# PKU-EPIC/GraspNeRF

Hardware: AMD Instinct MI355X
Metric: scenes/sec TSDF+render fwd, 6-view 40^3 grid (higher is better)
Workload: dtype f32

## Files before the change

graspnerf_amd/csrc/gnr_kernels.hip:

```cpp
#include <hip/hip_runtime.h>
#include <stdint.h>
#include <type_traits>

#include "gnr_layout.h"

#ifndef GNR_ABLATE
#define GNR_ABLATE 0
#endif

namespace gnr {

typedef float f4 __attribute__((ext_vector_type(4)));
typedef float f2 __attribute__((ext_vector_type(2)));

#define DEV __device__ __forceinline__

DEV f4 mfma16(float a, float b, f4 c) { return __builtin_amdgcn_mfma_f32_16x16x4f32(a, b, c, 0, 0, 0); }
DEV float elu1(float x) { return fmaxf(x, __builtin_amdgcn_fmed3f(__expf(x), 0.f, 1.f) - 1.f); }
constexpr float kLog2e = 1.4426950408889634f, kLn2 = 0.6931471805599453f;
#if GNR_ABLATE & 8
DEV float elu_s(float xs) { return xs; }
#else
DEV float elu_s(float xs) { return fmaxf(xs, fmaf(__builtin_amdgcn_fmed3f(__builtin_amdgcn_exp2f(xs), 0.f, 1.f), kLog2e, -kLog2e)); }
#endif
// ... 689 lines not shown
        return t < t_end - xcd * chunk ? xcd * chunk + t : -1;
#endif
    };
    auto locate = [&](int tile_, int& b_, int& ts_) {
        b_ = tile_ / tps;
        ts_ = tile_ - b_ * tps;
        b_ += a.b0;
        if (a.vol_res > 0) {
            const int R = a.vol_res, tpg = R >> 3, gpr = R >> 1;
            const int BX = R >> 2, GY = R >> 3, GB = BX * GY;
            const int sidx = ts_ / tpg, tin = ts_ - sidx * tpg;
            const int brick = sidx / GB, wi = sidx - brick * GB;
            const int bx = brick >> 2, by = brick & 3;
            ts_ = ((BX * bx + wi / GY) * gpr + GY * by + wi % GY) * tpg + tin;
        }
    };
    auto point_of = [&](int b_, int ts_) -> size_t { const int nr = ts_ * 16 + r; return (size_t)b_ * a.P + (nr < a.P ? nr : a.P - 1); };
    int tile = dyn ? resolve(grab()) : xcd * chunk + lblk * waves_per_block + wave;
    constexpr bool DPF = GNR_DESC_PREFETCH != 0 && !SAVE;
    f4 d0n = {0.f, 0.f, 0.f, 0.f}, d1n = d0n;
    bool have_nxt = false;
    for (; dyn ? tile >= 0 : tile < t_end;) {
        GNR_ITER_FENCE();
        unsigned tile_nxt = 0u;
        int tile_after = -1;
#if GNR_WAVE_CLOCK
        const unsigned long long wc_tt = wall_clock64();
#endif
        int b, ts;
        locate(tile, b, ts);
        const int n_raw = ts * 16 + r;
        const bool row_ok = n_raw < a.P;
        const int n = row_ok ? n_raw : a.P - 1;
        const size_t pt = (size_t)b * a.P + n;
        size_t opt = pt;
        if (RENDER && !SAVE && a.ray_perm) {
            const int s_ = n / a.perm_dn;
            opt = (size_t)b * a.P + (size_t)a.ray_perm[(size_t)b * a.perm_rn + s_] * a.perm_dn + (n - s_ * a.perm_dn);
        }
        float p[3], qd[3], lo, hi;
        {
            f4 d0, d1;
            if (DPF && have_nxt) { d0 = d0n; d1 = d1n; }
            else if (!RENDER && !SAVE && GNR_VOLUME_POINTS_INLINE != 0 && a.pts_R > 0) {
                const int R = a.pts_R;
                const float invR = 1.f / (float)R;
                const int col = (int)(((float)n + 0.5f) * invR), sz = n - col * R;
                const int ix = (int)(((float)col + 0.5f) * invR), iy = col - ix * R, iz = R - 1 - sz;
                const double vs = 0.3 / (double)R, hv = vs / 2;
                const float* bm = a.bbox_min + b * 3;
                d0 = (f4){(float)(ix * vs + hv) + bm[0], (float)(iy * vs + hv) + bm[1], (float)(iz * vs + hv) + bm[2], 0.f};
                d1 = (f4){0.f, 1.f, 0.005f, 0.005f};
            }
            else { d0 = reinterpret_cast<const f4*>(a.desc)[pt * 2]; d1 = reinterpret_cast<const f4*>(a.desc)[pt * 2 + 1]; }
            p[0] = d0.x; p[1] = d0.y; p[2] = d0.z; qd[0] = d0.w; qd[1] = d1.x; qd[2] = d1.y; lo = d1.z; hi = d1.w;
        }
        constexpr int VA = rows_a(V), VB = rows_b(V);
        float SA[VA][SW], SB[VB > 0 ? VB : 1][SW];
        auto S = [&](int v, int q) -> float& { return (VB == 0 || v < VA) ? SA[v < VA ? v : 0][q] : SB[v >= VA ? v - VA : 0][q]; };
#pragma unroll
        for (int k = 0; k < V; ++k)
#pragma unroll
#if GNR_ABLATE & 1
            for (int q = 0; q < SW; ++q) S(k, q) = p[0] * (float)(k * SW + q + 1);
#else
            for (int q = 0; q < SW; ++q) S(k, q) = 0.f;
#endif
        float msum = 0.f;
        unsigned vbits = 0;
#if GNR_ABLATE & 2
        ViewGeom vg0;
        project_view<true>(a.viewp + b * V * VIEWP_FLOATS, p, qd, a.H, a.W, vg0);
        const Taps t0 = make_taps(vg0.u, vg0.v, fsx, fsy, -0.5f, a.fh, a.fw);
        const Taps ti0 = make_taps(vg0.u, vg0.v, 1.f, 1.f, 0.f, a.H, a.W);
#endif

        auto phase1 = [&](auto& Q, const int v0) __attribute__((always_inline)) {
          constexpr int NQ = (int)(sizeof(Q) / sizeof(Q[0]));
#pragma unroll 1
          for (int v = v0; v < v0 + NQ; ++v) {
#if !(GNR_ABLATE & 1)
#pragma unroll
            for (int k = 0; k < NQ - 1; ++k)
#pragma unroll
                for (int q = 0; q < SW; ++q) Q[k][q] = Q[k + 1][q];
#endif
            GNR_ITER_FENCE();
            float (&Sv)[SW] = Q[NQ - 1];
            const int bv = b * V + v;
            const float* vp = a.viewp + bv * VIEWP_FLOATS;
            ViewGeom vg;
            Taps t, ti;
#if GNR_ABLATE & 2
            vg = vg0; t = t0; ti = ti0;
#elif GNR_COOP_PROJ
            {
                CoopOut co;
                project_coop(vp, lds + COOP_TAB + g * 8, (g & 1) * 16, (lane & 15) << 2, p, co);
                view_dir(vp, p, qd, vg.dd);
                vg.z = co.z; vg.m = co.m; t = co.f; ti = co.i;
            }
#else
            project_view<true>(vp, p, qd, a.H, a.W, vg);
            t = make_taps(vg.u, vg.v, fsx, fsy, -0.5f, a.fh, a.fw);
            ti = make_taps(vg.u, vg.v, 1.f, 1.f, 0.f, a.H, a.W);
#endif
            const float m = vg.m;
            msum += m;
            vbits |= (m != 0.f ? 1u : 0u) << v;
#if GNR_SKIP_MASKED
            if constexpr (!SAVE && RENDER) {
                if (__ballot(m != 0.f) == 0ull) {
#pragma unroll
                    for (int q = 0; q < SW; ++q) Sv[q] = 0.f;
                    if (a.dbg && g == 0 && row_ok) { a.dbg[pt * 32 + v] = 0.f; a.dbg[pt * 32 + 8 + v] = 0.f; }
                    continue;
                }
            }
#endif

            float FR[8], XI[9];
            {
                const float* fb = a.feat64 + (size_t)bv * a.fh * a.fw * 64 + 8 * g;
                const f4* q00 = reinterpret_cast<const f4*>(fb + (size_t)t.o00 * 64);
                const f4* q01 = reinterpret_cast<const f4*>(fb + (size_t)t.o01 * 64);
                const f4* q10 = reinterpret_cast<const f4*>(fb + (size_t)t.o10 * 64);
                const f4* q11 = reinterpret_cast<const f4*>(fb + (size_t)t.o11 * 64);
                const float w00 = t.w00 * m, w01 = t.w01 * m, w10 = t.w10 * m, w11 = t.w11 * m;
#pragma unroll
                for (int h = 0; h < 2; ++h) {
                    const f4 a0 = q00[h], a1 = q01[h], a2 = q10[h], a3 = q11[h];
                    const f4 c0 = q00[8 + h], c1 = q01[8 + h], c2 = q10[8 + h], c3 = q11[8 + h];
                    const f4 fr = a0 * w00 + a1 * w01 + a2 * w10 + a3 * w11;
                    const f4 fi = c0 * w00 + c1 * w01 + c2 * w10 + c3 * w11;
                    FR[4 * h] = fr.x; FR[4 * h + 1] = fr.y; FR[4 * h + 2] = fr.z; FR[4 * h + 3] = fr.w;
                    XI[4 * h] = fi.x; XI[4 * h + 1] = fi.y; XI[4 * h + 2] = fi.z; XI[4 * h + 3] = fi.w;
                }
                const float* ib = a.imgs + ((size_t)bv * 3 + min(g, 2)) * a.H * a.W;
                const float rgb = (ib[ti.o00] * ti.w00 + ib[ti.o01] * ti.w01 + ib[ti.o10] * ti.w10 + ib[ti.o11] * ti.w11) * m;
                XI[8] = g < 3 ? rgb : 0.f;
            }
            Sv[19] = XI[8];

            float o5[5];
            P8 frp;
            if constexpr (SP) frp = split8<0>(FR);
#pragma unroll
            for (int br = 0; br < 3; ++br) {
                f4 acc[2];
                float h1[8], h2[8];
                load_bias<2, LF>(lds + LO(pk::B_DEC1) + br * 32, g, acc);
                if constexpr (SP) mm16<1, 2, LF>(lds + LO(pk::DEC1) + br * frag_floats(8, 2), lane, &frp, acc);
                else mm<8, 2, 0, LF>(lds + LO(pk::DEC1) + br * frag_floats(8, 2), lane, FR, acc);
                elu_to<2, !SP>(acc, h1);
                load_bias<2, LF>(lds + LO(pk::B_DEC2) + br * 32, g, acc);
                if constexpr (SP) {
                    if constexpr (UA) { const P8U hp = split8u<0>(h1); mm16u<1, 2, LF, true>(lds + LO(pk::DEC2) + br * frag_floats(8, 2), lane, &hp, acc, &msum); }
                    else { const P8 hp = split8<0>(h1); mm16<1, 2, LF, true>(lds + LO(pk::DEC2) + br * frag_floats(8, 2), lane, &hp, acc, &msum); }
                }
                else mm<8, 2, 0, LF>(lds + LO(pk::DEC2) + br * frag_floats(8, 2), lane, h1, acc);
                elu_to<2, !SP || UA>(acc, h2);
                if (br < 2) {
                    o5[2 * br] = gsum(dot8(lds + LO(pk::T_DEC3) + (2 * br) * 32, g, h2)) + lds[LO(pk::T_DEC3_B) + 2 * br];
                    o5[2 * br + 1] = gsum(dot8(lds + LO(pk::T_DEC3) + (2 * br + 1) * 32, g, h2)) + lds[LO(pk::T_DEC3_B) + 2 * br + 1];
                } else {
                    o5[4] = gsum(dot8(lds + LO(pk::T_DEC3) + 4 * 32, g, h2)) + lds[LO(pk::T_DEC3_B) + 4];
                }
            }
            float hit, vis;
            {
                const bool m1 = (g & 1) != 0, far_edge = g >= 2;
                const float meang = softplus1(m1 ? o5[1] : o5[0]);
                const float varg = softplus1(m1 ? o5[3] : o5[2]) + 0.05f;
                const float mix = sigmoid1(m1 ? -o5[4] : o5[4]);
                const float dinv = -rcp1(fmaxf(vg.z, 1e-5f));
                const float dhat = (dinv - vp[15]) * vp[17];
                const float edge = far_edge ? dhat + hi : dhat - lo;
                float cg = 0.5f + 0.5f * tanh1((edge - meang) * varg);
                if constexpr (USEVIS) {
                    f4 acc[2];
                    float h1[8], h2[8];
                    load_bias<2, LF>(lds + LO(pk::B_DECV1), g, acc);
                    if constexpr (SP) mm16<1, 2, LF>(lds + LO(pk::DECV1), lane, &frp, acc);
                    else mm<8, 2, 0, LF>(lds + LO(pk::DECV1), lane, FR, acc);
                    elu_to<2, !SP>(acc, h1);
                    load_bias<2, LF>(lds + LO(pk::B_DECV2), g, acc);
                    if constexpr (SP) {
                        if constexpr (UA) { const P8U hp = split8u<0>(h1); mm16u<1, 2, LF, true>(lds + LO(pk::DECV2), lane, &hp, acc, &msum); }
                        else { const P8 hp = split8<0>(h1); mm16<1, 2, LF, true>(lds + LO(pk::DECV2), lane, &hp, acc, &msum); }
                    }
                    else mm<8, 2, 0, LF>(lds + LO(pk::DECV2), lane, h1, acc);
                    elu_to<2, !SP || UA>(acc, h2);
                    const float pv = sigmoid1(gsum(dot8(lds + LO(pk::T_DECV3), g, h2)) + lds[LO(pk::T_VIS)]);
                    cg *= pv;
                }
                const float mc = mix * cg;
                vis = gsum(far_edge ? 0.f : mix - mc) * m;
                hit = gsum(far_edge ? mc : -mc) * m;
            }
            {
                f4 acc[2];
                float e1[8];
                load_bias<2, LF>(lds + LO(pk::B_PE1), g, acc);
                if constexpr (SP) mm16<1, 2, LF>(lds + LO(pk::PE1), lane, &frp, acc);
                else mm<8, 2, 0, LF>(lds + LO(pk::PE1), lane, FR, acc);
                const float extra[1] = {g == 0 ? (hit - 0.5f) * 2.f : (g == 1 ? (vis - 0.5f) * 2.f : 0.f)};
                mm<1, 2, 8, LF>(lds + LO(pk::PE1), lane, extra, acc);
#pragma unroll
                for (int nb = 0; nb < 2; ++nb) {
                    e1[nb * 4 + 0] = fmaxf(acc[nb].x, 0.f); e1[nb * 4 + 1] = fmaxf(acc[nb].y, 0.f);
                    e1[nb * 4 + 2] = fmaxf(acc[nb].z, 0.f); e1[nb * 4 + 3] = fmaxf(acc[nb].w, 0.f);
                }
                if constexpr (EP) p8_store(split8<0>(e1), &Sv[9]);
                else {
#pragma unroll
                    for (int j = 0; j < 8; ++j) Sv[9 + j] = e1[j];
                }
            }
            {
                f4 acc1[1], acc3[3];
                float d1[4], df[12];
                load_bias<1, LF>(lds + LO(pk::B_RDF1), g, acc1);
                const float ddg[1] = {g == 0 ? vg.dd[0] : (g == 1 ? vg.dd[1] : (g == 2 ? vg.dd[2] : vg.dd[3]))};
                mm<1, 1, 0, LF>(lds + LO(pk::RDF1), lane, ddg, acc1);
                elu_to<1, true>(acc1, d1);
                load_bias<3, LF>(lds + LO(pk::B_RDF2), g, acc3);
#if GNR_RDF2_PAIRS
                if constexpr (SP && !USEVIS) { const P8 dp = split8z<0, 4>(d1); mm16<1, 3, LF>(lds + pk::c16_off(pk::DECV1), lane, &dp, acc3); }
                else
#endif
                mm<4, 3, 0, LF>(lds + LO(pk::RDF2), lane, d1, acc3);
                elu_to<3, true>(acc3, df);
#pragma unroll
                for (int j = 0; j < 9; ++j) Sv[j] = fmaf(df[j], kLn2, XI[j]);
            }
            {
                f4 acc1[1];
                float e[8], n1[4];
#pragma unroll
                for (int j = 0; j < 8; ++j) e[j] = Sv[9 + j];
                load_bias<1, LF>(lds + LO(pk::B_NR1), g, acc1);
                if constexpr (SP) { const P8 ep = EP ? p8_load(e) : split8<0>(e); mm16<1, 1, LF, true>(lds + LO(pk::NR1), lane, &ep, acc1, &msum); }
                else mm<8, 1, 0, LF>(lds + LO(pk::NR1), lane, e, acc1);
                elu_to<1, !SP>(acc1, n1);
                Sv[17] = sigmoid1(gsum(dot4(lds + LO(pk::T_NR2), g, n1)) + lds[LO(pk::T_SCAL) + 0]);
            }
            Sv[18] = m;
            if (SAVE && a.save1) {
                float* sp = a.save1 + (((size_t)b * tps + ts) * V + v) * 19 * 64 + lane;
#pragma unroll
                for (int q = 0; q < 19; ++q) sp[q * 64] = Sv[q];
            }
            if (a.dbg && g == 0 && row_ok) { a.dbg[pt * 32 + v] = hit; a.dbg[pt * 32 + 8 + v] = vis; }
          }
        };
        phase1(SA, 0);
        if constexpr (VB > 0) phase1(SB, VA);
#if GNR_WAVE_CLOCK
        const unsigned long long wc_p1 = wall_clock64();
#endif

        float SV[36];
        const float inv_msum = rcp1(msum + 1e-8f);
        {
#pragma unroll
            for (int j = 0; j < 9; ++j) {
                float mu0 = 0.f, mu1 = 0.f;
#pragma unroll
                for (int v = 0; v < V; ++v) {
                    const float w = S(v, 18) * inv_msum;
                    mu0 += S(v, j) * (S(v, 17) * w);
                    mu1 += S(v, j) * w;
                }
                float va0 = 0.f, va1 = 0.f;
#pragma unroll
                for (int v = 0; v < V; ++v) {
                    const float w = S(v, 18) * inv_msum;
                    const float d0 = S(v, j) - mu0, d1 = S(v, j) - mu1;
                    va0 += (S(v, 17) * w) * d0 * d0;
                    va1 += w * d1 * d1;
                }
                SV[j] = mu0; SV[9 + j] = va0; SV[18 + j] = mu1; SV[27 + j] = va1;
            }
        }
        f4 G[4];
        load_bias<4, LF>(lds + LO(pk::B_HOIST), g, G);
        if constexpr (SP) {
            const P8 sp[5] = {split8<0>(SV), split8<8>(SV), split8<16>(SV), split8<24>(SV), split8z<32, 4>(SV)};
            mm16<5, 4, LF, true>(lds + LO(pk::HOIST), lane, sp, G, &msum);
        } else mm<36, 4, 0, LF>(lds + LO(pk::HOIST), lane, SV, G);
        if (SAVE && a.saveG) {
            float* sp = a.saveG + ((size_t)b * tps + ts) * 17 * 64 + lane;
#pragma unroll
            for (int nb = 0; nb < 4; ++nb) {
                sp[(4 * nb) * 64] = G[nb].x; sp[(4 * nb + 1) * 64] = G[nb].y; sp[(4 * nb + 2) * 64] = G[nb].z; sp[(4 * nb + 3) * 64] = G[nb].w;
            }
            sp[16 * 64] = inv_msum;
        }

#if GNR_WAVE_CLOCK
        const unsigned long long wc_p2 = wall_clock64();
#endif
        float vsum = 0.f;
        auto phase2 = [&](auto& Q, const int v0) __attribute__((always_inline)) {
          constexpr int NQ = (int)(sizeof(Q) / sizeof(Q[0]));
#pragma unroll 1
          for (int v = v0; v < v0 + NQ; ++v) {
            constexpr int RN = 20;
            float Rv[RN];
#pragma unroll
            for (int j = 0; j < RN; ++j) Rv[j] = Q[0][j];
#if !(GNR_ABLATE & 1)
#pragma unroll
            for (int k = 0; k < NQ - 1; ++k)
#pragma unroll
                for (int q = 0; q < SW; ++q) Q[k][q] = Q[k + 1][q];
#endif
            GNR_ITER_FENCE();
            float X[9], E[8];
#pragma unroll
            for (int j = 0; j < 9; ++j) X[j] = Rv[j];
#pragma unroll
            for (int j = 0; j < 8; ++j) E[j] = Rv[9 + j];
            const float m = Rv[18];
            const float w = m * inv_msum;
#if GNR_SKIP_MASKED
            if constexpr (!SAVE && RENDER) {
                if (__ballot(m != 0.f) == 0ull) {
#pragma unroll
                    for (int j = 0; j < 9; ++j) Q[NQ - 1][j] = 0.f;
                    Q[NQ - 1][9] = RENDER ? -1e9f : 0.f;
                    Q[NQ - 1][19] = Rv[19];
                    if (a.dbg && g == 0 && row_ok) a.dbg[pt * 32 + 16 + v] = 0.f;
                    continue;
                }
            }
#endif
            float Hh[8];
            {
                f4 acc4[4] = {G[0], G[1], G[2], G[3]};
                float b1[16];
                if constexpr (SP) {
                    const float x8[1] = {X[8]};
                    mm<1, 4, 0, LF>(lds + LO(pk::BASE1) + 2 * pk::k32_floats(4), lane, x8, acc4);
                    const P8 xe[2] = {split8<0>(X), EP ? p8_load(E) : split8<0>(E)};
                    mm16<2, 4, LF, true>(lds + LO(pk::BASE1), lane, xe, acc4, &msum);
                } else {
                    mm<9, 4, 0, LF>(lds + LO(pk::BASE1), lane, X, acc4);
                    mm<8, 4, 9, LF>(lds + LO(pk::BASE1), lane, E, acc4);
                }
                elu_to<4, !SP>(acc4, b1);
                f4 acc[2];
                load_bias<2, LF>(lds + LO(pk::B_BASE2), g, acc);
                if constexpr (SP) {
                    if constexpr (UA) { const P8U bp[2] = {split8u<0>(b1), split8u<8>(b1)}; mm16u<2, 2, LF, true>(lds + LO(pk::BASE2), lane, bp, acc, &msum); }
                    else { const P8 bp[2] = {split8<0>(b1), split8<8>(b1)}; mm16<2, 2, LF, true>(lds + LO(pk::BASE2), lane, bp, acc, &msum); }
                }
                else mm<16, 2, 0, LF>(lds + LO(pk::BASE2), lane, b1, acc);
                elu_to<2, !SP || UA>(acc, Hh);
            }
            float vis1;
            {
                f4 acc[2];
                float xin[8], v1[8], res[8];
#pragma unroll
                for (int j = 0; j < 8; ++j) xin[j] = Hh[j] * w;
                load_bias<2, LF>(lds + LO(pk::B_VIS1), g, acc);
                if constexpr (SP) {
                    if constexpr (UA) { const P8U xp = split8u<0>(xin); mm16u<1, 2, LF, true>(lds + LO(pk::VIS1), lane, &xp, acc, &msum); }
                    else { const P8 xp = split8<0>(xin); mm16<1, 2, LF, true>(lds + LO(pk::VIS1), lane, &xp, acc, &msum); }
                }
                else mm<8, 2, 0, LF>(lds + LO(pk::VIS1), lane, xin, acc);
                elu_to<2, !SP || UA>(acc, v1);
                load_bias<2, LF>(lds + LO(pk::B_VIS2), g, acc);
                if constexpr (SP) {
                    if constexpr (UA) { const P8U vp8 = split8u<0>(v1); mm16u<1, 2, LF, true>(lds + LO(pk::VIS2), lane, &vp8, acc, &msum); }
                    else { const P8 vp8 = split8<0>(v1); mm16<1, 2, LF, true>(lds + LO(pk::VIS2), lane, &vp8, acc, &msum); }
                }
                else mm<8, 2, 0, LF>(lds + LO(pk::VIS2), lane, v1, acc);
                elu_to<2, !SP || UA>(acc, res);
                const float logit = elu1(gsum(dot8(lds + LO(pk::T_VIS2R), g, v1)) + lds[LO(pk::T_SCAL) + 1]);
                vis1 = sigmoid1(logit) * m;
#pragma unroll
                for (int j = 0; j < 8; ++j) Hh[j] += res[j];
            }
            float v2;
            {
                f4 acc[2];
                float xin[8], t1[8];
#pragma unroll
                for (int j = 0; j < 8; ++j) xin[j] = Hh[j] * vis1;
                load_bias<2, LF>(lds + LO(pk::B_VISB1), g, acc);
                if constexpr (SP) {
                    if constexpr (UA) { const P8U xp = split8u<0>(xin); mm16u<1, 2, LF, true>(lds + LO(pk::VISB1), lane, &xp, acc, &msum); }
                    else { const P8 xp = split8<0>(xin); mm16<1, 2, LF, true>(lds + LO(pk::VISB1), lane, &xp, acc, &msum); }
                }
                else mm<8, 2, 0, LF>(lds + LO(pk::VISB1), lane, xin, acc);
                elu_to<2, !SP || UA>(acc, t1);
                v2 = sigmoid1(gsum(dot8(lds + LO(pk::T_VISB2), g, t1)) + lds[LO(pk::T_SCAL) + 2]) * m;
            }
            vsum += v2;
            float clog = 0.f;
            if constexpr (RENDER) {
                const float* vp = a.viewp + (b * V + v) * VIEWP_FLOATS;
                ViewGeom vg;
                project_view<true>(vp, p, qd, a.H, a.W, vg);
                f4 acc1[1];
                float c1[4], c2[4];
                load_bias<1, LF>(lds + LO(pk::B_RGB1), g, acc1);
                const float ex[2] = {g == 0 ? v2 : (g == 1 ? vg.dd[0] : (g == 2 ? vg.dd[1] : vg.dd[2])), g == 0 ? vg.dd[3] : 0.f};
                mm<2, 1, 8, LF>(lds + LO(pk::RGB1), lane, ex, acc1);
                if constexpr (SP) { const P8 hp = split8<0>(Hh); mm16<1, 1, LF, true>(lds + LO(pk::RGB1), lane, &hp, acc1, &msum); }
                else mm<8, 1, 0, LF>(lds + LO(pk::RGB1), lane, Hh, acc1);
                elu_to<1, !SP>(acc1, c1);
                load_bias<1, LF>(lds + LO(pk::B_RGB2), g, acc1);
                mm<4, 1, 0, LF>(lds + LO(pk::RGB2), lane, c1, acc1);
                elu_to<1, true>(acc1, c2);
                clog = gsum(dot4(lds + LO(pk::T_RGB3), g, c2)) + lds[LO(pk::T_SCAL) + 3];
                if (m == 0.f) clog = -1e9f;
            }
            float Ov[10];
#pragma unroll
            for (int j = 0; j < 8; ++j) Ov[j] = Hh[j];
            Ov[8] = v2;
            Ov[9] = clog;
            if (SAVE && a.save2) {
                constexpr int S2W = RENDER ? 11 : 9;
                float* sp = a.save2 + (((size_t)b * tps + ts) * V + v) * S2W * 64 + lane;
#pragma unroll
                for (int q = 0; q < (S2W < 10 ? S2W : 10); ++q) sp[q * 64] = Ov[q];
                if constexpr (RENDER) sp[10 * 64] = Rv[RN - 1];
            }
#pragma unroll
            for (int j = 0; j < 10; ++j) Q[NQ - 1][j] = Ov[j];
            Q[NQ - 1][19] = Rv[19];
            if (a.dbg && g == 0 && row_ok) a.dbg[pt * 32 + 16 + v] = v2;
          }
        };
        phase2(SA, 0);
        if constexpr (VB > 0) phase2(SB, VA);
#if GNR_WAVE_CLOCK
        const unsigned long long wc_p3 = wall_clock64();
#endif
        if (dyn) {
            bool more = true;
#if GNR_TAIL_OLD_ONLY
            if (wave >= 4) more = (t_end - tile) > (GNR_TAIL_OLD_ONLY * nlblk * waves_per_block) / 4;
#endif
            tile_nxt = more ? grab() : 0x7fffffffu;
        }
        if constexpr (DPF) {
            tile_after = dyn ? resolve(tile_nxt) : tile + nlblk * waves_per_block;
            have_nxt = dyn ? tile_after >= 0 : tile_after < t_end;
            if (have_nxt) {
                int bn, tsn;
                locate(tile_after, bn, tsn);
                const size_t ptn = point_of(bn, tsn);
                d0n = reinterpret_cast<const f4*>(a.desc)[ptn * 2]; d1n = reinterpret_cast<const f4*>(a.desc)[ptn * 2 + 1];
            }
        }

        float Z[23];
        float wbar = 0.f;
        {
            const float inv_vsum = rcp1(vsum + 1e-8f);
#pragma unroll
            for (int v = 0; v < V; ++v) wbar += S(v, 8) * inv_vsum;
            wbar *= (1.f / (float)V);
#pragma unroll
            for (int j = 0; j < 8; ++j) {
                float mu = 0.f, va = 0.f;
#pragma unroll
                for (int v = 0; v < V; ++v) mu += S(v, j) * (S(v, 8) * inv_vsum);
#pragma unroll
                for (int v = 0; v < V; ++v) { const float d = S(v, j) - mu; va += (S(v, 8) * inv_vsum) * d * d; }
                Z[j] = mu; Z[8 + j] = va;
            }
        }
        if constexpr (RENDER) {
            float cmax = -3.0e38f;
#pragma unroll
            for (int v = 0; v < V; ++v) cmax = fmaxf(cmax, S(v, 9));
            float den = 0.f, num = 0.f;
#pragma unroll
            for (int v = 0; v < V; ++v) { const float e = __expf(S(v, 9) - cmax); den += e; num += S(v, 19) * e; }
            if (g < 3 && row_ok) a.colors[opt * 3 + g] = num * rcp1(den);
        }
        if (SAVE && a.saveZ) {
            float* sp = a.saveZ + ((size_t)b * tps + ts) * 18 * 64 + lane;
#pragma unroll
            for (int q = 0; q < 16; ++q) sp[q * 64] = Z[q];
            sp[16 * 64] = wbar; sp[17 * 64] = msum;
        }
        {
            const float pc = g == 1 ? p[0] : (g == 2 ? p[1] : p[2]);
            float s1, c1, s2, c2, s4, c4;
            sincos_octaves(pc, s1, c1, s2, c2, s4, c4);
            const bool g0 = g == 0;
            Z[16] = g0 ? wbar : pc; Z[17] = g0 ? 0.f : s1; Z[18] = g0 ? 0.f : c1; Z[19] = g0 ? 0.f : s2;
            Z[20] = g0 ? 0.f : c2; Z[21] = g0 ? 0.f : s4; Z[22] = g0 ? 0.f : c4;
        }
        f4 U[4];
        float u64[16];
        load_bias<4, LF>(lds + LO(pk::B_GEO1), g, U);
        if constexpr (SP) {
            const P8 zp[3] = {split8<0>(Z), split8<8>(Z), split8z<16, 7>(Z)};
            mm16<3, 4, LF, true>(lds + LO(pk::GEO1), lane, zp, U, &msum);
        } else mm<23, 4, 0, LF>(lds + LO(pk::GEO1), lane, Z, U);
        elu_to<4, !SP>(U, u64);
        f4 g16[1];
        load_bias<1, LF>(lds + LO(pk::B_GEO2), g, g16);
        if constexpr (SP) { const P8 up[2] = {split8<0>(u64), split8<8>(u64)}; mm16<2, 1, LF, true>(lds + LO(pk::GEO2), lane, up, g16, &msum); }
        else mm<16, 1, 0, LF>(lds + LO(pk::GEO2), lane, u64, g16);
        float gg[4];
        elu_to<1, !SP>(g16, gg);

        if constexpr (SP && GNR_RANGE_GUARD != 0) range_tripped |= __ballot(msum != msum) != 0;
        if (row_ok) {
            float* rec = a.rec + pt * REC;
            const f4 gv = {gg[0] * kLn2, gg[1] * kLn2, gg[2] * kLn2, gg[3] * kLn2};
            reinterpret_cast<f4*>(rec)[g] = gv;
            if constexpr (RENDER) {
#pragma unroll
                for (int nb = 0; nb < 4; ++nb) {
                    const f4 uv = {u64[nb * 4] * kLn2, u64[nb * 4 + 1] * kLn2, u64[nb * 4 + 2] * kLn2, u64[nb * 4 + 3] * kLn2};
                    reinterpret_cast<f4*>(rec + 16 + 16 * nb)[g] = uv;
                }
                if (g == 0) rec[80] = msum;
            } else {
                if (g == 0) rec[16] = msum;
            }
            if (a.vmask && g == 0) a.vmask[opt] = (unsigned char)vbits;
            if (a.dbg && g == 0) {
                float* d = a.dbg + pt * 32;
                d[24] = msum; d[25] = wbar; d[26] = Z[0] * kLn2; d[27] = Z[8] * kLn2 * kLn2; d[28] = SV[8]; d[29] = G[0].x * kLn2; d[30] = gg[0] * kLn2; d[31] = vsum;
            }
        }
#if GNR_WAVE_CLOCK
        if constexpr (SP && !SAVE) { const unsigned long long wc_e = wall_clock64(); ++wc_n; wc_ph[0] += wc_p1 - wc_tt; wc_ph[1] += wc_p2 - wc_p1; wc_ph[2] += wc_p3 - wc_p2; wc_ph[3] += wc_e - wc_p3;
            if (lane == 0 && tile < (1 << 17)) g_tile_clock[RENDER ? 1 : 0][tile] = (unsigned)(wc_e - wc_tt); }
#endif
#if GNR_DYN_CTR_INC
        if (dyn) asm volatile("" : "+v"(tile_nxt));
#endif
        if constexpr (DPF) tile = have_nxt ? tile_after : (dyn ? -1 : t_end);
        else tile = dyn ? resolve(tile_nxt) : tile + nlblk * waves_per_block;
    }
    if (dyn && lane == 0) {
        if (atomicAdd(a.tile_ctr + 8, 1u) == gridDim.x * (unsigned)waves_per_block - 1u) {
#pragma unroll
            for (int x = 0; x < 9; ++x) atomicExch(a.tile_ctr + x, 0u);
        }
    }
#if GNR_WAVE_CLOCK
    if constexpr (SP && !SAVE) {
        if (lane == 0 && !a.only_if_flagged && blockIdx.x * 8 + wave < 4096) {
            unsigned long long* w = g_wave_clock[RENDER ? 1 : 0][blockIdx.x * 8 + wave];
            w[0] = wc_t0; w[1] = wc_t1; w[2] = wall_clock64(); w[3] = wc_n;
            w[4] = wc_ph[0]; w[5] = wc_ph[1]; w[6] = wc_ph[2]; w[7] = wc_ph[3];
        }
    }
#endif
    if constexpr (SP) {
        if (range_tripped && lane == 0) {
            if (a.range_launch) atomicOr(a.range_launch, 2u);
            else if (a.range_flag) atomicOr(a.range_flag, 2u);
        }
    }
}

#undef LO

struct RayArgs {
    const float* wpk;
    const float* rec;
    const float* desc;
    const float* depth;
    const float* colors;
    const float* que_dr;
    const unsigned char* vmask_pts;
    int nrays, dn, rays_per_scene;
    int slots, rays_per_block, ray_stride;
    float* volume;
    unsigned char* vmask_out;
    float *sdf, *alpha, *hit, *pix, *rdepth, *gerr_part, *grad;
    unsigned char* rmask;
    int view_num, point_num;
    float* fine_depth; int* fine_inds; int fdn;
    const float* fine_u;
    unsigned* range_word;
    const unsigned* only_if;
    const int* ray_perm;
};

namespace rt {
constexpr int W = MAX_DN_FWD;
constexpr int TF = 0;
constexpr int RED = W;
constexpr int HP = 7 * W;
constexpr int DN = 8 * W;
constexpr int PD = 9 * W;
constexpr int CD = 10 * W;
constexpr int CE = 11 * W + 8;
constexpr int FD = 12 * W + 16;
constexpr int END = 13 * W + 16;
}

DEV void head_logits(const float (&q)[16], const float* __restrict__ Kj, bool ok, float (&s)[4]) {
#pragma unroll
    for (int h = 0; h < 4; ++h) {
        const f4 k = reinterpret_cast<const f4*>(Kj)[h];
        const float d = 0.5f * (q[4 * h] * k.x + q[4 * h + 1] * k.y + q[4 * h + 2] * k.z + q[4 * h + 3] * k.w);
        s[h] = ok ? d : -1e9f;
    }
}

DEV void head_logits_s(const float (&qs)[16], const float* __restrict__ Kj, float (&s)[4]) {
#pragma unroll
    for (int h = 0; h < 4; ++h) {
        const f4 k = reinterpret_cast<const f4*>(Kj)[h];
        s[h] = qs[4 * h] * k.x + qs[4 * h + 1] * k.y + qs[4 * h + 2] * k.z + qs[4 * h + 3] * k.w;
    }
}

#ifndef GNR_RAY_SEED
#define GNR_RAY_SEED 1
#endif
template <bool SD>
DEV void head_logits_shifted(const float (&qs)[16], const float* __restrict__ Kj, const float (&shift)[4], float (&s)[4]) {
#pragma unroll
    for (int h = 0; h < 4; ++h) {
        const f4 k = reinterpret_cast<const f4*>(Kj)[h];
        if constexpr (SD && GNR_RAY_SEED)
            s[h] = fmaf(qs[4 * h + 3], k.w, fmaf(qs[4 * h + 2], k.z, fmaf(qs[4 * h + 1], k.y, fmaf(qs[4 * h], k.x, -shift[h]))));
        else
            s[h] = (qs[4 * h] * k.x + qs[4 * h + 1] * k.y + qs[4 * h + 2] * k.z + qs[4 * h + 3] * k.w) - shift[h];
    }
}
template <bool SD = true>
DEV float dot4_minus(float a0, float a1, float a2, float a3, const f4& b, float c) {
    if constexpr (SD && GNR_RAY_SEED) return fmaf(a3, b.w, fmaf(a2, b.z, fmaf(a1, b.y, fmaf(a0, b.x, -c))));
    else return (a0 * b.x + a1 * b.y + a2 * b.z + a3 * b.w) - c;
}

#ifndef GNR_RAY_UNROLL
#define GNR_RAY_UNROLL 1
#endif
#ifndef GNR_RAY_BLOCKS
#define GNR_RAY_BLOCKS 3
#endif
constexpr int ray_per(bool render) { return render ? (GNR_RAY_BLOCKS >= 3 ? 44 : 80) : 36; }
#ifndef GNR_RAY_GEO_MFMA
#define GNR_RAY_GEO_MFMA (GNR_RAY_BLOCKS >= 3)
#endif
DEV void wave_sync() {
    __builtin_amdgcn_fence(__ATOMIC_RELEASE, "wavefront");
    __builtin_amdgcn_wave_barrier();
    __builtin_amdgcn_fence(__ATOMIC_ACQUIRE, "wavefront");
}
template <bool RENDER, bool MM = (GNR_RAY_GEO_MFMA != 0)>
__global__ __launch_bounds__(256, (RENDER ? GNR_RAY_BLOCKS : 2)) void k_ray(RayArgs a) {
    if constexpr (RENDER && !MM) {
        if (a.only_if && (__builtin_nontemporal_load(a.only_if) & 2u) == 0u) return;
    }
    extern __shared__ __attribute__((aligned(16))) float sm[];
    const int dn = a.dn, S = a.slots, rpb = a.rays_per_block;
    int rl = (int)threadIdx.x / S;
    const int slot = (int)threadIdx.x - rl * S;
    const bool in_blk = rl < rpb;
    rl = min(rl, rpb - 1);
    const int ray_u = blockIdx.x * rpb + rl;
    const bool rvalid = in_blk && ray_u < a.nrays;
    const int ray = min(ray_u, a.nrays - 1);
    const bool act = rvalid && slot < dn;
    const int i = min(slot, dn - 1);
    constexpr bool OVL = RENDER && GNR_RAY_BLOCKS >= 3;
    float* sc = sm + (size_t)rl * a.ray_stride;
    float* Kb = sc;
    float* Vb = sc + dn * 16;
    float* KN = sc + dn * 32;
    constexpr int KNS = 4;
    float* Qb = OVL ? sc : sc + dn * 36;
    float* Ob = OVL ? sc + dn * 16 : sc + dn * 52;
    float* St = OVL ? sc + dn * 32 : sc + dn * 68;
    (void)Qb; (void)St; (void)Ob;
    const size_t pt = (size_t)ray * dn + i;
    int oray = ray;
    if (RENDER && a.ray_perm) oray = (ray / a.rays_per_scene) * a.rays_per_scene + a.ray_perm[ray];
    const size_t opt = (size_t)oray * dn + i;
    (void)opt;
    constexpr int REC = RENDER ? REC_RAY : REC_VOL;
    const float* rec = a.rec + pt * REC;
    const float* W = a.wpk;
    constexpr int UB = GNR_RAY_UNROLL;
    constexpr int UA = RENDER ? UB : 4;

    float g16[16], t[16];
    {
        const f4* r4 = reinterpret_cast<const f4*>(rec);
        const f4* pe = reinterpret_cast<const f4*>(W + pk::R_PE + i * 16);
#pragma unroll
        for (int q = 0; q < 4; ++q) {
            const f4 x = r4[q], e = pe[q];
            g16[4 * q] = x.x; g16[4 * q + 1] = x.y; g16[4 * q + 2] = x.z; g16[4 * q + 3] = x.w;
            t[4 * q] = x.x + e.x; t[4 * q + 1] = x.y + e.y; t[4 * q + 2] = x.z + e.z; t[4 * q + 3] = x.w + e.w;
        }
    }
    const float nvalid = rec[RENDER ? 80 : 16];
    const bool rowok = nvalid > 1.f;

    float q[16], kk[16], vv[16];
#pragma unroll
    for (int f = 0; f < 16; ++f) {
        float sq = 0.f, sk = 0.f, sv = 0.f;
#pragma unroll
        for (int c = 0; c < 16; ++c) {
            sq = fmaf(W[pk::R_WQ + f * 16 + c], t[c], sq);
            sk = fmaf(W[pk::R_WK + f * 16 + c], t[c], sk);
            sv = fmaf(W[pk::R_WV + f * 16 + c], t[c], sv);
        }
        q[f] = sq; kk[f] = sk; vv[f] = sv;
    }
    float qs[16];
#pragma unroll
    for (int f = 0; f < 16; ++f) qs[f] = rowok ? q[f] * (0.5f * kLog2e) : 0.f;
    if (act) {
#pragma unroll
        for (int c = 0; c < 4; ++c) {
            const f4 k4 = {kk[4 * c], kk[4 * c + 1], kk[4 * c + 2], kk[4 * c + 3]};
            const f4 v4 = {vv[4 * c], vv[4 * c + 1], vv[4 * c + 2], vv[4 * c + 3]};
            reinterpret_cast<f4*>(Kb + i * 16)[c] = k4;
            reinterpret_cast<f4*>(Vb + i * 16)[c] = v4;
            KN[i * KNS + c] = k4.x * k4.x + k4.y * k4.y + k4.z * k4.z + k4.w * k4.w;
            if constexpr (RENDER && !OVL) {
                const f4 q4 = {qs[4 * c], qs[4 * c + 1], qs[4 * c + 2], qs[4 * c + 3]};
                reinterpret_cast<f4*>(Qb + i * 16)[c] = q4;
            }
        }
    }
// ... 553 lines not shown
```

Before: 4999.

## Interleave two views' MLP chains in phase2 to hide MFMA latency

Splits the per-view phase-2 body into a reusable function and adds a paired path that processes two views at once. Each layer's MFMA for one view is interleaved with the elementwise prep of the other, and sched_group_barrier hints place VALU work in the MFMA shadows. The paired path is only enabled for the non-save, non-render variant with the UA and EP layouts and an even queue length. It raises register pressure and ties performance to compiler scheduling hints. It also duplicates the MLP logic, which must stay in sync with the original path.

Result: faster. 5079, median of 6 (+1.6%).

```diff
diff --git a/graspnerf_amd/csrc/gnr_kernels.hip b/graspnerf_amd/csrc/gnr_kernels.hip
--- a/graspnerf_amd/csrc/gnr_kernels.hip
+++ b/graspnerf_amd/csrc/gnr_kernels.hip
@@ -1015,21 +1015,8 @@
         const unsigned long long wc_p2 = wall_clock64();
 #endif
         float vsum = 0.f;
-        auto phase2 = [&](auto& Q, const int v0) __attribute__((always_inline)) {
-          constexpr int NQ = (int)(sizeof(Q) / sizeof(Q[0]));
-#pragma unroll 1
-          for (int v = v0; v < v0 + NQ; ++v) {
-            constexpr int RN = 20;
-            float Rv[RN];
-#pragma unroll
-            for (int j = 0; j < RN; ++j) Rv[j] = Q[0][j];
-#if !(GNR_ABLATE & 1)
-#pragma unroll
-            for (int k = 0; k < NQ - 1; ++k)
-#pragma unroll
-                for (int q = 0; q < SW; ++q) Q[k][q] = Q[k + 1][q];
-#endif
-            GNR_ITER_FENCE();
+        auto view2 = [&](const float (&Rv)[SW], const int v, float (&Out)[SW]) __attribute__((always_inline)) -> float {
+            constexpr int RN = SW;
             float X[9], E[8];
 #pragma unroll
             for (int j = 0; j < 9; ++j) X[j] = Rv[j];
@@ -1037,18 +1024,6 @@
             for (int j = 0; j < 8; ++j) E[j] = Rv[9 + j];
             const float m = Rv[18];
             const float w = m * inv_msum;
-#if GNR_SKIP_MASKED
-            if constexpr (!SAVE && RENDER) {
-                if (__ballot(m != 0.f) == 0ull) {
-#pragma unroll
-                    for (int j = 0; j < 9; ++j) Q[NQ - 1][j] = 0.f;
-                    Q[NQ - 1][9] = RENDER ? -1e9f : 0.f;
-                    Q[NQ - 1][19] = Rv[19];
-                    if (a.dbg && g == 0 && row_ok) a.dbg[pt * 32 + 16 + v] = 0.f;
-                    continue;
-                }
-            }
-#endif
             float Hh[8];
             {
                 f4 acc4[4] = {G[0], G[1], G[2], G[3]};
@@ -1112,7 +1087,6 @@
                 elu_to<2, !SP || UA>(acc, t1);
                 v2 = sigmoid1(gsum(dot8(lds + LO(pk::T_VISB2), g, t1)) + lds[LO(pk::T_SCAL) + 2]) * m;
             }
-            vsum += v2;
             float clog = 0.f;
             if constexpr (RENDER) {
                 const float* vp = a.viewp + (b * V + v) * VIEWP_FLOATS;
@@ -1145,9 +1119,147 @@
                 if constexpr (RENDER) sp[10 * 64] = Rv[RN - 1];
             }
 #pragma unroll
-            for (int j = 0; j < 10; ++j) Q[NQ - 1][j] = Ov[j];
-            Q[NQ - 1][19] = Rv[19];
-            if (a.dbg && g == 0 && row_ok) a.dbg[pt * 32 + 16 + v] = v2;
+            for (int j = 0; j < 10; ++j) Out[j] = Ov[j];
+            Out[19] = Rv[19];
+            return v2;
+        };
+        auto view2p = [&](const float (*Rv)[SW], float (*Out)[SW], float* v2) __attribute__((always_inline)) {
+            constexpr int NL = 5;
+            float m[2], w[2], Hh[2][8], v1[2][8], vis1[2];
+            f4 acc4[2][4], acc[2][2];
+            P8 xe[2][2];
+            P8U up[2][2];
+            float x8[2][1];
+#pragma unroll
+            for (int c = 0; c < 2; ++c) { m[c] = Rv[c][18]; w[c] = m[c] * inv_msum; }
+            auto prep = [&](const int c, const int k) __attribute__((always_inline)) {
+                if (k == 0) {
+                    float X[9], E[8];
+#pragma unroll
+                    for (int j = 0; j < 9; ++j) X[j] = Rv[c][j];
+#pragma unroll
+                    for (int j = 0; j < 8; ++j) E[j] = Rv[c][9 + j];
+                    x8[c][0] = X[8];
+                    xe[c][0] = split8<0>(X); xe[c][1] = p8_load(E);
+#pragma unroll
+                    for (int nb = 0; nb < 4; ++nb) acc4[c][nb] = G[nb];
+                } else if (k == 1) {
+                    float b1[16];
+                    elu_to<4, false>(acc4[c], b1);
+                    up[c][0] = split8u<0>(b1); up[c][1] = split8u<8>(b1);
+                    load_bias<2, LF>(lds + LO(pk::B_BASE2), g, acc[c]);
+                } else if (k == 2) {
+                    elu_to<2, true>(acc[c], Hh[c]);
+                    float xin[8];
+#pragma unroll
+                    for (int j = 0; j < 8; ++j) xin[j] = Hh[c][j] * w[c];
+                    up[c][0] = split8u<0>(xin);
+                    load_bias<2, LF>(lds + LO(pk::B_VIS1), g, acc[c]);
+                } else if (k == 3) {
+                    elu_to<2, true>(acc[c], v1[c]);
+                    up[c][0] = split8u<0>(v1[c]);
+                    load_bias<2, LF>(lds + LO(pk::B_VIS2), g, acc[c]);
+                } else if (k == 4) {
+                    float res[8];
+                    elu_to<2, true>(acc[c], res);
+                    const float logit = elu1(gsum(dot8(lds + LO(pk::T_VIS2R), g, v1[c])) + lds[LO(pk::T_SCAL) + 1]);
+                    vis1[c] = sigmoid1(logit) * m[c];
+                    float xin[8];
+#pragma unroll
+                    for (int j = 0; j < 8; ++j) { Hh[c][j] += res[j]; xin[j] = Hh[c][j] * vis1[c]; }
+                    up[c][0] = split8u<0>(xin);
+                    load_bias<2, LF>(lds + LO(pk::B_VISB1), g, acc[c]);
+                } else {
+                    float t1[8];
+                    elu_to<2, true>(acc[c], t1);
+                    v2[c] = sigmoid1(gsum(dot8(lds + LO(pk::T_VISB2), g, t1)) + lds[LO(pk::T_SCAL) + 2]) * m[c];
+                }
+            };
+            auto mfma = [&](const int c, const int k) __attribute__((always_inline)) {
+                if (k == 0) {
+                    mm<1, 4, 0, LF>(lds + LO(pk::BASE1) + 2 * pk::k32_floats(4), lane, x8[c], acc4[c]);
+                    mm16<2, 4, LF, true>(lds + LO(pk::BASE1), lane, xe[c], acc4[c], &msum);
+                } else if (k == 1) mm16u<2, 2, LF, true>(lds + LO(pk::BASE2), lane, up[c], acc[c], &msum);
+                else if (k == 2) mm16u<1, 2, LF, true>(lds + LO(pk::VIS1), lane, up[c], acc[c], &msum);
+                else if (k == 3) mm16u<1, 2, LF, true>(lds + LO(pk::VIS2), lane, up[c], acc[c], &msum);
+                else mm16u<1, 2, LF, true>(lds + LO(pk::VISB1), lane, up[c], acc[c], &msum);
+            };
+            auto shadows = [&](const int k) __attribute__((always_inline)) {
+                const int n = k == 0 ? 28 : (k == 1 ? 12 : 6);
+                for (int i = 0; i < n; ++i) {
+                    __builtin_amdgcn_sched_group_barrier(0x008, 1, 0);
+                    __builtin_amdgcn_sched_group_barrier(0x002, 2, 0);
+                }
+                __builtin_amdgcn_sched_barrier(0);
+            };
+            prep(0, 0);
+            __builtin_amdgcn_sched_barrier(0);
+#pragma unroll
+            for (int k = 0; k < NL; ++k) {
+                mfma(0, k); prep(1, k); shadows(k);
+                mfma(1, k); prep(0, k + 1); shadows(k);
+            }
+            prep(1, NL);
+#pragma unroll
+            for (int c = 0; c < 2; ++c) {
+#pragma unroll
+                for (int j = 0; j < 8; ++j) Out[c][j] = Hh[c][j];
+                Out[c][8] = v2[c];
+                Out[c][9] = 0.f;
+                Out[c][19] = Rv[c][19];
+            }
+        };
+        auto skip2 = [&](const float (&Rv)[SW], float (&Out)[SW]) __attribute__((always_inline)) {
+#pragma unroll
+            for (int j = 0; j < 9; ++j) Out[j] = 0.f;
+            Out[9] = RENDER ? -1e9f : 0.f;
+            Out[19] = Rv[19];
+        };
+        constexpr bool SKIP2 = GNR_SKIP_MASKED != 0 && !SAVE && RENDER;
+        auto phase2 = [&](auto& Q, const int v0) __attribute__((always_inline)) {
+          constexpr int NQ = (int)(sizeof(Q) / sizeof(Q[0]));
+          constexpr bool PAIR2 = UA && EP && !SAVE && !RENDER && NQ % 2 == 0;
+          if constexpr (PAIR2) {
+#pragma unroll 1
+            for (int v = v0; v < v0 + NQ; v += 2) {
+              float RP[2][SW];
+#pragma unroll
+              for (int j = 0; j < SW; ++j) { RP[0][j] = Q[0][j]; RP[1][j] = Q[1][j]; }
+#if !(GNR_ABLATE & 1)
+#pragma unroll
+              for (int k = 0; k < NQ - 2; ++k)
+#pragma unroll
+                  for (int q = 0; q < SW; ++q) Q[k][q] = Q[k + 2][q];
+#endif
+              GNR_ITER_FENCE();
+              float v2p[2];
+              view2p(RP, &Q[NQ - 2], v2p);
+              vsum += v2p[0];
+              vsum += v2p[1];
+              if (a.dbg && g == 0 && row_ok) { a.dbg[pt * 32 + 16 + v] = v2p[0]; a.dbg[pt * 32 + 17 + v] = v2p[1]; }
+            }
+          } else {
+#pragma unroll 1
+            for (int v = v0; v < v0 + NQ; ++v) {
+              float Rv[SW];
+#pragma unroll
+              for (int j = 0; j < SW; ++j) Rv[j] = Q[0][j];
+#if !(GNR_ABLATE & 1)
+#pragma unroll
+              for (int k = 0; k < NQ - 1; ++k)
+#pragma unroll
+                  for (int q = 0; q < SW; ++q) Q[k][q] = Q[k + 1][q];
+#endif
+              GNR_ITER_FENCE();
+              if (SKIP2 && __ballot(Rv[18] != 0.f) == 0ull) {
+                  skip2(Rv, Q[NQ - 1]);
+                  if (a.dbg && g == 0 && row_ok) a.dbg[pt * 32 + 16 + v] = 0.f;
+                  continue;
+              }
+              const float v2 = view2(Rv, v, Q[NQ - 1]);
+              vsum += v2;
+              if (a.dbg && g == 0 && row_ok) a.dbg[pt * 32 + 16 + v] = v2;
+            }
           }
         };
         phase2(SA, 0);
```
